# AIR-DISCOVER/Omni-PQ

Measured on AMD Instinct MI355X. Metric: scenes/sec fwd+bwd, 40k-pt ScanNet clouds, batch 8/GPU, higher is better.
Workload: dtype bf16; 1 GPU; BASELINE configs[1]: PQ_Transformer fwd+bwd, 40000-pt synthetic room scenes, batch 8/GPU, 3 input channels; global_batch=8, points=40000, parallelism=dp1, loss=sum of output means (SURVEY 8d)

## Files before the change

### include/omnipq_attn.h

```cpp
#ifndef OMNIPQ_ATTN_H
#define OMNIPQ_ATTN_H
#include "omnipq_pointops.h"

#ifdef __cplusplus
extern "C" {
#endif

int omnipq_attn_fwd(int N, int H, int L, int S, int D, const void *q, const void *k, const void *v, void *o,
                    const long long *strides, float *lse2, float dropout_p, const unsigned long long *seed_ptr,
                    unsigned salt, void *stream);

int omnipq_attn_bwd(int N, int H, int L, int S, int D, const void *q, const void *k, const void *v, const void *o,
                    const void *d_o, const long long *strides, const float *lse2, float *delta, void *dq, void *dk,
                    void *dv, const long long *grad_strides, float dropout_p, const unsigned long long *seed_ptr,
                    unsigned salt, void *stream);

int omnipq_attn_dropout_mask(int N, int H, int L, int S, float dropout_p, const unsigned long long *seed_ptr,
                             unsigned salt, unsigned char *mask, void *stream);

void omnipq_attn_block_map(int mode);

#ifdef __cplusplus
}
#endif
#endif
```

### omni-pq_amd/csrc/attention.hip

```cpp
#include "common.h"
#include "omnipq_attn.h"

namespace omnipq {

typedef float f32x16 __attribute__((ext_vector_type(16)));

constexpr int ATT_DMAX = 48;
constexpr int ATT_PITCH = 56;

struct AttnArgs {
  int N, H, L, S, D;
  long long q_sl, q_sn, k_sl, k_sn, v_sl, v_sn, o_sl, o_sn;
  float scale, scale_log2;
  float keep_inv;
  unsigned drop_thresh;
  unsigned salt;
  int xcd_map;
  const unsigned long long *seed_ptr;
};

__device__ __forceinline__ unsigned drop_seed(const AttnArgs &g) {
  if (!g.drop_thresh) return 0u;
  const unsigned long long s = *g.seed_ptr * 0x9E3779B97F4A7C15ull + 0xD1B54A32D192ED03ull * (g.salt + 1u);
  return (unsigned)(s >> 32) ^ (unsigned)s;
// ... 30 lines not shown
}

__device__ __forceinline__ float bf_lo(unsigned w) { return e16_lo(w); }
__device__ __forceinline__ float bf_hi(unsigned w) { return e16_hi(w); }

__device__ __forceinline__ float frag_dot(e16x8 a, e16x8 b) {
  const uint4 x = __builtin_bit_cast(uint4, a), y = __builtin_bit_cast(uint4, b);
  float s = bf_lo(x.x) * bf_lo(y.x) + bf_hi(x.x) * bf_hi(y.x);
  s += bf_lo(x.y) * bf_lo(y.y) + bf_hi(x.y) * bf_hi(y.y);
  s += bf_lo(x.z) * bf_lo(y.z) + bf_hi(x.z) * bf_hi(y.z);
  s += bf_lo(x.w) * bf_lo(y.w) + bf_hi(x.w) * bf_hi(y.w);
  return s;
}

__device__ __forceinline__ e16x8 pack_regs(const float *p, int j2) {
  e16x8 f;
#pragma unroll
  for (int e = 0; e < 8; ++e) f[e] = (e16_t)p[8 * j2 + e];
  return f;
}

constexpr int ATT_NP = 6;
constexpr int ATT_AREA = 33 * ATT_PITCH;
struct StagePlan {
  unsigned voff[ATT_NP];
  int lds[ATT_NP];
};

__device__ __forceinline__ StagePlan stage_plan(int D, int lane, long long s_tok) {
  StagePlan sp;
  const int ppr = D >> 2;
#pragma unroll
  for (int i = 0; i < ATT_NP; ++i) {
    const int id = lane + 64 * i;
    const int tok = id / ppr, off = (id - tok * ppr) * 4;
    const bool has = id < 32 * ppr;
    sp.voff[i] = has ? (unsigned)(tok * (int)s_tok + off) * 2u : ATT_OOB;
    sp.lds[i] = has ? tok * ATT_PITCH + off : 32 * ATT_PITCH;
  }
  return sp;
}

struct StageRegs {
  v2u v[ATT_NP];
};

__device__ __forceinline__ StageRegs stage_load(const StagePlan &sp, rsrc_t block) {
  StageRegs r;
#pragma unroll
  for (int i = 0; i < ATT_NP; ++i) r.v[i] = att_load8(block, sp.voff[i]);
  return r;
}

__device__ __forceinline__ void stage_store(const StagePlan &sp, const StageRegs &r, e16_t *lds) {
#pragma unroll
  for (int i = 0; i < ATT_NP; ++i) *reinterpret_cast<v2u *>(lds + sp.lds[i]) = r.v[i];
}

__device__ __forceinline__ void stage_clear(e16_t *lds, int areas, int lane) {
  for (int o = lane * 4; o < areas * ATT_AREA; o += 256) *reinterpret_cast<v2u *>(lds + o) = v2u{0u, 0u};
}

__device__ __forceinline__ e16x8 frag_lds_tok(const e16_t *lds, int row, int j, int h) {
  return *reinterpret_cast<const e16x8 *>(lds + row * ATT_PITCH + 16 * j + 8 * h);
}

typedef short v4s __attribute__((ext_vector_type(4)));
typedef __attribute__((address_space(3))) v4s lds_v4s;

__device__ __forceinline__ e16x8 frag_chan(const e16_t *lds, int t, int j2, int h, int lane) {
  const int grp = lane >> 4, l16 = lane & 15;
  int c0 = 32 * t + 16 * (grp & 1);
  c0 = c0 + 16 <= ATT_DMAX ? c0 : ATT_DMAX - 16;
  const e16_t *p = lds + (16 * j2 + 4 * h + (l16 >> 2)) * ATT_PITCH + c0 + (l16 & 3) * 4;
  const v4s lo = __builtin_amdgcn_ds_read_tr16_b64_v4i16((lds_v4s *)p);
  const v4s hi = __builtin_amdgcn_ds_read_tr16_b64_v4i16((lds_v4s *)(p + 8 * ATT_PITCH));
  return __builtin_bit_cast(e16x8, __builtin_shufflevector(lo, hi, 0, 1, 2, 3, 4, 5, 6, 7));
}

__device__ __forceinline__ float fast_exp2(float x) { return __builtin_amdgcn_exp2f(x); }

__device__ __forceinline__ float xor32(float v) { return __shfl_xor(v, 32, 64); }

__device__ __forceinline__ void att_block(const AttnArgs &g, int &blk, int &nh) {
  const int gx = (int)gridDim.x, gy = (int)gridDim.y;
  blk = (int)blockIdx.x, nh = (int)blockIdx.y;
  if (g.xcd_map && (gy & 7) == 0) {
    const int id = blk + gx * nh, slot = id >> 3;
    nh = (id & 7) + 8 * (slot / gx);
    blk = slot % gx;
  }
}

#define MFMA(a, b, c) mfma_e16_32x32x16(a, b, c)

__global__ __launch_bounds__(256) void attn_fwd_kernel(AttnArgs g, const e16_t *__restrict__ Q,
                                                      const e16_t *__restrict__ K, const e16_t *__restrict__ V,
                                                      e16_t *__restrict__ O, float *__restrict__ lse2) {
  __shared__ __attribute__((aligned(16))) unsigned char smem[4 * 64 * 33 * 4 + 4 * 32 * 4 * 2];
  const int tid = (int)threadIdx.x, lane = tid & 63, wave = __builtin_amdgcn_readfirstlane(tid >> 6), h = lane >> 5, ql = lane & 31;
  int blk, nh;
  att_block(g, blk, nh);
  const int n = nh / g.H, hd = nh - n * g.H;
  const int q0 = blk * 32, q = q0 + ql;
  const e16_t *Qb = Q + n * g.q_sn + hd * g.D, *Kb = K + n * g.k_sn + hd * g.D, *Vb = V + n * g.v_sn + hd * g.D;
  e16_t *ks = reinterpret_cast<e16_t *>(smem) + wave * 2 * ATT_AREA, *vs = ks + ATT_AREA;
  stage_clear(ks, 2, lane);

  e16x8 qf[3];
  {
    const rsrc_t rq = att_rsrc(Qb, g.q_sl, q0, g.L, g.D);
#pragma unroll
    for (int j = 0; j < 3; ++j) qf[j] = frag_tok(rq, (unsigned)(ql * (int)g.q_sl) * 2u, j, h, g.D);
  }

  const unsigned seed = drop_seed(g);
  float m = -1e30f, lsum = 0.f;
  f32x16 acc[2];
#pragma unroll
  for (int t = 0; t < 2; ++t)
#pragma unroll
    for (int r = 0; r < 16; ++r) acc[t][r] = 0.f;

  const int nkb = (g.S + 31) >> 5, iters = (nkb + 3) >> 2;
  const StagePlan spk = stage_plan(g.D, lane, g.k_sl), spv = stage_plan(g.D, lane, g.v_sl);
  StageRegs kn = stage_load(spk, att_rsrc(Kb, g.k_sl, wave * 32, g.S, g.D));
  StageRegs vn = stage_load(spv, att_rsrc(Vb, g.v_sl, wave * 32, g.S, g.D));
  for (int it = 0; it < iters; ++it) {
    const int k0 = (it * 4 + wave) * 32;
    const StageRegs kc = kn, vc = vn;
    if (it + 1 < iters) {
      kn = stage_load(spk, att_rsrc(Kb, g.k_sl, k0 + 128, g.S, g.D));
      vn = stage_load(spv, att_rsrc(Vb, g.v_sl, k0 + 128, g.S, g.D));
    }
    __builtin_amdgcn_fence(__ATOMIC_ACQ_REL, "wavefront");
    __builtin_amdgcn_wave_barrier();
    stage_store(spk, kc, ks);
    stage_store(spv, vc, vs);
    __builtin_amdgcn_fence(__ATOMIC_ACQ_REL, "wavefront");
    __builtin_amdgcn_wave_barrier();
    f32x16 st;
#pragma unroll
    for (int r = 0; r < 16; ++r) st[r] = 0.f;
#pragma unroll
    for (int j = 0; j < 3; ++j) st = MFMA(frag_lds_tok(ks, ql, j, h), qf[j], st);
    float p[16], bm = -1e30f;
    const bool full = k0 + 32 <= g.S;
    if (full) {
#pragma unroll
      for (int r = 0; r < 16; ++r) bm = fmaxf(bm, st[r]);
      bm *= g.scale_log2;
    } else {
#pragma unroll
      for (int r = 0; r < 16; ++r) {
        const bool ok = k0 + acc_row(r, h) < g.S;
        p[r] = ok ? st[r] * g.scale_log2 : -1e30f;
        bm = fmaxf(bm, p[r]);
      }
    }
    bm = fmaxf(bm, xor32(bm));
    const float m_new = fmaxf(m, bm);
    const float alpha = fast_exp2(m - m_new);
    float rs = 0.f;
    if (full) {
#pragma unroll
      for (int r = 0; r < 16; ++r) {
        p[r] = fast_exp2(__builtin_fmaf(st[r], g.scale_log2, -m_new));
        rs += p[r];
      }
    } else {
#pragma unroll
      for (int r = 0; r < 16; ++r) {
        const bool ok = k0 + acc_row(r, h) < g.S;
        p[r] = ok ? fast_exp2(p[r] - m_new) : 0.f;
        rs += p[r];
      }
    }
    rs += xor32(rs);
    lsum = lsum * alpha + rs;
    if (__builtin_amdgcn_ballot_w64(m_new != m) != 0) {
#pragma unroll
      for (int t = 0; t < 2; ++t)
#pragma unroll
        for (int r = 0; r < 16; ++r) acc[t][r] *= alpha;
    }
    m = m_new;
    if (g.drop_thresh) {
      const unsigned base = ((unsigned)nh * (unsigned)g.L + (unsigned)q) * (unsigned)g.S + (unsigned)k0 + seed + 4u * h;
#pragma unroll
      for (int r = 0; r < 16; ++r)
        p[r] = drop_hash_mix(base + (unsigned)acc_row(r, 0)) >= g.drop_thresh ? p[r] * g.keep_inv : 0.f;
    }
    __builtin_amdgcn_fence(__ATOMIC_ACQ_REL, "wavefront");
    __builtin_amdgcn_wave_barrier();
#pragma unroll
    for (int j2 = 0; j2 < 2; ++j2) {
      const e16x8 pf = pack_regs(p, j2);
#pragma unroll
      for (int t = 0; t < 2; ++t) acc[t] = MFMA(frag_chan(vs, t, j2, h, lane), pf, acc[t]);
    }
  }

  __syncthreads();
  float *ms = reinterpret_cast<float *>(smem + 4 * 64 * 33 * 4);
  float *comb = reinterpret_cast<float *>(smem);
  if (h == 0) ms[wave * 32 + ql] = m;
  __syncthreads();
  const float mstar = fmaxf(fmaxf(ms[ql], ms[32 + ql]), fmaxf(ms[64 + ql], ms[96 + ql]));
  const float f = fast_exp2(m - mstar);
  if (h == 0) ms[128 + wave * 32 + ql] = lsum * f;
#pragma unroll
  for (int t = 0; t < 2; ++t)
#pragma unroll
    for (int r = 0; r < 16; ++r) comb[(wave * 64 + 32 * t + acc_row(r, h)) * 33 + ql] = acc[t][r] * f;
  __syncthreads();
  for (int idx = tid; idx < 32 * g.D; idx += 256) {
    const int qq = idx / g.D, d = idx - qq * g.D;
    if (q0 + qq < g.L) {
      const float l = ms[128 + qq] + ms[160 + qq] + ms[192 + qq] + ms[224 + qq];
      const float o = comb[(0 * 64 + d) * 33 + qq] + comb[(1 * 64 + d) * 33 + qq] + comb[(2 * 64 + d) * 33 + qq] +
                      comb[(3 * 64 + d) * 33 + qq];
      O[(long long)(q0 + qq) * g.o_sl + n * g.o_sn + hd * g.D + d] = (e16_t)(o / l);
    }
  }
  if (tid < 32 && q0 + tid < g.L) {
    const float l = ms[128 + tid] + ms[160 + tid] + ms[192 + tid] + ms[224 + tid];
    const float ms_ = fmaxf(fmaxf(ms[tid], ms[32 + tid]), fmaxf(ms[64 + tid], ms[96 + tid]));
    lse2[(long long)nh * g.L + q0 + tid] = ms_ + log2f(l);
  }
}

__global__ __launch_bounds__(256) void attn_bwd_dq_kernel(AttnArgs g, const e16_t *__restrict__ Q,
                                                         const e16_t *__restrict__ K, const e16_t *__restrict__ V,
                                                         const e16_t *__restrict__ O, const e16_t *__restrict__ dO,
                                                         const float *__restrict__ lse2, float *__restrict__ delta,
                                                         e16_t *__restrict__ dQ, long long dq_sl, long long dq_sn) {
  __shared__ __attribute__((aligned(16))) unsigned char smem[4 * 64 * 33 * 4];
  const int tid = (int)threadIdx.x, lane = tid & 63, wave = __builtin_amdgcn_readfirstlane(tid >> 6), h = lane >> 5, ql = lane & 31;
  int blk, nh;
  att_block(g, blk, nh);
  const int n = nh / g.H, hd = nh - n * g.H;
  const int q0 = blk * 32, q = q0 + ql;
  const bool qv = q < g.L;
  const e16_t *Qb = Q + n * g.q_sn + hd * g.D, *Kb = K + n * g.k_sn + hd * g.D, *Vb = V + n * g.v_sn + hd * g.D;
  const e16_t *Ob = O + n * g.o_sn + hd * g.D, *dOb = dO + n * g.o_sn + hd * g.D;
  e16_t *ks = reinterpret_cast<e16_t *>(smem) + wave * 2 * ATT_AREA, *vs = ks + ATT_AREA;
  stage_clear(ks, 2, lane);

  e16x8 qf[3], dof[3];
  float dl = 0.f;
  {
    const rsrc_t rq = att_rsrc(Qb, g.q_sl, q0, g.L, g.D), ro = att_rsrc(Ob, g.o_sl, q0, g.L, g.D);
    const rsrc_t rdo = att_rsrc(dOb, g.o_sl, q0, g.L, g.D);
    const unsigned qoff = (unsigned)(ql * (int)g.q_sl) * 2u, ooff = (unsigned)(ql * (int)g.o_sl) * 2u;
#pragma unroll
    for (int j = 0; j < 3; ++j) {
      qf[j] = frag_tok(rq, qoff, j, h, g.D);
      dof[j] = frag_tok(rdo, ooff, j, h, g.D);
      dl += frag_dot(dof[j], frag_tok(ro, ooff, j, h, g.D));
    }
  }
  dl += xor32(dl);
  if (wave == 0 && h == 0 && qv) delta[(long long)nh * g.L + q] = dl;
  const float lse = qv ? lse2[(long long)nh * g.L + q] : 0.f;

  const unsigned seed = drop_seed(g);
  f32x16 acc[2];
#pragma unroll
  for (int t = 0; t < 2; ++t)
#pragma unroll
    for (int r = 0; r < 16; ++r) acc[t][r] = 0.f;

  const int nkb = (g.S + 31) >> 5, iters = (nkb + 3) >> 2;
  const StagePlan spk = stage_plan(g.D, lane, g.k_sl), spv = stage_plan(g.D, lane, g.v_sl);
  StageRegs kn = stage_load(spk, att_rsrc(Kb, g.k_sl, wave * 32, g.S, g.D));
  StageRegs vn = stage_load(spv, att_rsrc(Vb, g.v_sl, wave * 32, g.S, g.D));
  for (int it = 0; it < iters; ++it) {
    const int k0 = (it * 4 + wave) * 32;
    const StageRegs kc = kn, vc = vn;
    if (it + 1 < iters) {
      kn = stage_load(spk, att_rsrc(Kb, g.k_sl, k0 + 128, g.S, g.D));
      vn = stage_load(spv, att_rsrc(Vb, g.v_sl, k0 + 128, g.S, g.D));
    }
    __builtin_amdgcn_fence(__ATOMIC_ACQ_REL, "wavefront");
    __builtin_amdgcn_wave_barrier();
    stage_store(spk, kc, ks);
    stage_store(spv, vc, vs);
    __builtin_amdgcn_fence(__ATOMIC_ACQ_REL, "wavefront");
    __builtin_amdgcn_wave_barrier();
    f32x16 st, dp;
#pragma unroll
    for (int r = 0; r < 16; ++r) st[r] = dp[r] = 0.f;
#pragma unroll
    for (int j = 0; j < 3; ++j) {
      st = MFMA(frag_lds_tok(ks, ql, j, h), qf[j], st);
      dp = MFMA(frag_lds_tok(vs, ql, j, h), dof[j], dp);
    }
    float ds[16];
    const unsigned base = ((unsigned)nh * (unsigned)g.L + (unsigned)q) * (unsigned)g.S + (unsigned)k0 + seed + 4u * h;
    const bool full = q0 + 32 <= g.L && k0 + 32 <= g.S;
#pragma unroll
    for (int r = 0; r < 16; ++r) ds[r] = fast_exp2(__builtin_fmaf(st[r], g.scale_log2, -lse));
    if (!full) {
#pragma unroll
      for (int r = 0; r < 16; ++r) ds[r] = (qv && k0 + acc_row(r, h) < g.S) ? ds[r] : 0.f;
    }
    if (g.drop_thresh) {
#pragma unroll
      for (int r = 0; r < 16; ++r)
        dp[r] = drop_hash_mix(base + (unsigned)acc_row(r, 0)) >= g.drop_thresh ? dp[r] * g.keep_inv : 0.f;
    }
#pragma unroll
    for (int r = 0; r < 16; ++r) ds[r] *= dp[r] - dl;
#pragma unroll
    for (int j2 = 0; j2 < 2; ++j2) {
      const e16x8 df = pack_regs(ds, j2);
#pragma unroll
      for (int t = 0; t < 2; ++t) acc[t] = MFMA(frag_chan(ks, t, j2, h, lane), df, acc[t]);
    }
  }
  __syncthreads();
  float *comb = reinterpret_cast<float *>(smem);
#pragma unroll
  for (int t = 0; t < 2; ++t)
#pragma unroll
    for (int r = 0; r < 16; ++r) comb[(wave * 64 + 32 * t + acc_row(r, h)) * 33 + ql] = acc[t][r];
  __syncthreads();
  for (int idx = tid; idx < 32 * g.D; idx += 256) {
    const int qq = idx / g.D, d = idx - qq * g.D;
    if (q0 + qq < g.L) {
      const float v = comb[(0 * 64 + d) * 33 + qq] + comb[(1 * 64 + d) * 33 + qq] + comb[(2 * 64 + d) * 33 + qq] +
                      comb[(3 * 64 + d) * 33 + qq];
      dQ[(long long)(q0 + qq) * dq_sl + n * dq_sn + hd * g.D + d] = (e16_t)(v * g.scale);
    }
  }
}

__global__ __launch_bounds__(256) void attn_bwd_dkdv_kernel(AttnArgs g, const e16_t *__restrict__ Q,
                                                           const e16_t *__restrict__ K, const e16_t *__restrict__ V,
                                                           const e16_t *__restrict__ dO, const float *__restrict__ lse2,
                                                           const float *__restrict__ delta, e16_t *__restrict__ dK,
                                                           long long dk_sl, long long dk_sn, e16_t *__restrict__ dV,
                                                           long long dv_sl, long long dv_sn) {
  __shared__ __attribute__((aligned(16))) e16_t qs[2 * ATT_AREA];
  __shared__ float rowv[64];
  const int tid = (int)threadIdx.x, lane = tid & 63, wave = __builtin_amdgcn_readfirstlane(tid >> 6), h = lane >> 5, kl = lane & 31;
  int blk, nh;
  att_block(g, blk, nh);
  const int n = nh / g.H, hd = nh - n * g.H;
  const int kb0 = blk * 128, k0 = kb0 + wave * 32, key = k0 + kl;
  const bool kv = key < g.S;
  const e16_t *Qb = Q + n * g.q_sn + hd * g.D, *Kb = K + n * g.k_sn + hd * g.D, *Vb = V + n * g.v_sn + hd * g.D;
  const e16_t *dOb = dO + n * g.o_sn + hd * g.D;
  e16_t *dos = qs + ATT_AREA;
  for (int o = tid * 4; o < 2 * ATT_AREA; o += 1024) *reinterpret_cast<v2u *>(qs + o) = v2u{0u, 0u};

  e16x8 kf[3], vf[3];
  {
    const rsrc_t rk = att_rsrc(Kb, g.k_sl, kb0, g.S, g.D), rv = att_rsrc(Vb, g.v_sl, kb0, g.S, g.D);
    const unsigned koff = (unsigned)((wave * 32 + kl) * (int)g.k_sl) * 2u, voff = (unsigned)((wave * 32 + kl) * (int)g.v_sl) * 2u;
#pragma unroll
    for (int j = 0; j < 3; ++j) {
      kf[j] = frag_tok(rk, koff, j, h, g.D);
      vf[j] = frag_tok(rv, voff, j, h, g.D);
    }
  }
  const unsigned seed = drop_seed(g);
  f32x16 accv[2], acck[2];
#pragma unroll
  for (int t = 0; t < 2; ++t)
#pragma unroll
    for (int r = 0; r < 16; ++r) accv[t][r] = acck[t][r] = 0.f;

  const int ppr = g.D >> 2;
  unsigned qvo[2], dvo[2];
  int plds[2];
#pragma unroll
  for (int i = 0; i < 2; ++i) {
    const int id = tid + 256 * i, tok = id / ppr, off = (id - tok * ppr) * 4;
    const bool has = id < 32 * ppr;
    qvo[i] = has ? (unsigned)(tok * (int)g.q_sl + off) * 2u : ATT_OOB;
    dvo[i] = has ? (unsigned)(tok * (int)g.o_sl + off) * 2u : ATT_OOB;
    plds[i] = has ? tok * ATT_PITCH + off : 32 * ATT_PITCH;
  }
  const float *rowsrc = (tid < 32 ? lse2 : delta) + (long long)nh * g.L;
  v2u qn[2], dn[2];
  float rown = 0.f;
  auto fetch = [&](int q0) {
    const rsrc_t rq = att_rsrc(Qb, g.q_sl, q0, g.L, g.D), rdo = att_rsrc(dOb, g.o_sl, q0, g.L, g.D);
#pragma unroll
    for (int i = 0; i < 2; ++i) {
      qn[i] = att_load8(rq, qvo[i]);
      dn[i] = att_load8(rdo, dvo[i]);
    }
    rown = (tid < 64 && q0 + (tid & 31) < g.L) ? rowsrc[q0 + (tid & 31)] : 0.f;
  };
  fetch(0);
  const int nqb = (g.L + 31) >> 5;
  __syncthreads();
  for (int it = 0; it < nqb; ++it) {
    const int q0 = it * 32;
    v2u qc[2], dc[2];
#pragma unroll
    for (int i = 0; i < 2; ++i) qc[i] = qn[i], dc[i] = dn[i];
    const float rowc = rown;
    if (it + 1 < nqb) fetch(q0 + 32);
    __syncthreads();
#pragma unroll
    for (int i = 0; i < 2; ++i) {
      *reinterpret_cast<v2u *>(qs + plds[i]) = qc[i];
      *reinterpret_cast<v2u *>(dos + plds[i]) = dc[i];
    }
    if (tid < 64) rowv[tid] = rowc;
    __syncthreads();
    f32x16 s, dp;
#pragma unroll
    for (int r = 0; r < 16; ++r) s[r] = dp[r] = 0.f;
#pragma unroll
    for (int j = 0; j < 3; ++j) {
      s = MFMA(frag_lds_tok(qs, kl, j, h), kf[j], s);
      dp = MFMA(frag_lds_tok(dos, kl, j, h), vf[j], dp);
    }
    float pt[16], ds[16];
    const bool full = q0 + 32 <= g.L && k0 + 32 <= g.S;
    const unsigned hbase = ((unsigned)nh * (unsigned)g.L + (unsigned)(q0 + 4 * h)) * (unsigned)g.S + (unsigned)key + seed;
#pragma unroll
    for (int r = 0; r < 16; ++r) pt[r] = fast_exp2(__builtin_fmaf(s[r], g.scale_log2, -rowv[acc_row(r, h)]));
    if (!full) {
#pragma unroll
      for (int r = 0; r < 16; ++r) pt[r] = (kv && q0 + acc_row(r, h) < g.L) ? pt[r] : 0.f;
    }
#pragma unroll
    for (int r = 0; r < 16; ++r) ds[r] = pt[r];
    if (g.drop_thresh) {
#pragma unroll
      for (int r = 0; r < 16; ++r) {
        const float km = drop_hash_mix(hbase + (unsigned)acc_row(r, 0) * (unsigned)g.S) >= g.drop_thresh ? g.keep_inv : 0.f;
        dp[r] *= km;
        pt[r] *= km;
      }
    }
#pragma unroll
    for (int r = 0; r < 16; ++r) ds[r] *= dp[r] - rowv[32 + acc_row(r, h)];
#pragma unroll
    for (int j2 = 0; j2 < 2; ++j2) {
      const e16x8 pf = pack_regs(pt, j2), df = pack_regs(ds, j2);
#pragma unroll
      for (int t = 0; t < 2; ++t) {
        accv[t] = MFMA(pf, frag_chan(dos, t, j2, h, lane), accv[t]);
        acck[t] = MFMA(df, frag_chan(qs, t, j2, h, lane), acck[t]);
      }
    }
  }
#pragma unroll
  for (int t = 0; t < 2; ++t) {
    const int d = 32 * t + kl;
    if (d < g.D) {
#pragma unroll
      for (int r = 0; r < 16; ++r) {
        const int kk = k0 + acc_row(r, h);
        if (kk < g.S) {
          dV[(long long)kk * dv_sl + n * dv_sn + hd * g.D + d] = (e16_t)accv[t][r];
          dK[(long long)kk * dk_sl + n * dk_sn + hd * g.D + d] = (e16_t)(acck[t][r] * g.scale);
        }
      }
    }
  }
}

__global__ void attn_mask_kernel(AttnArgs g, unsigned char *__restrict__ mask) {
  const long long total = (long long)g.N * g.H * g.L * g.S;
  const unsigned seed = drop_seed(g);
  for (long long i = (long long)blockIdx.x * blockDim.x + threadIdx.x; i < total; i += (long long)gridDim.x * blockDim.x)
    mask[i] = !g.drop_thresh || drop_hash((unsigned)i, seed) >= g.drop_thresh;
}

static int g_attn_xcd_map = 1;

static int token_strides_ok(const long long *strides, int n, int L, int S, int D) {
  const long long tok = L > S ? L : S;
  for (int i = 0; i < 2 * n; i += 2) {
    const long long sl = strides[i];
    if (sl < 0) return OMNIPQ_EINVAL;
    if (((tok - 1) * sl + D) * 2 >= (1ll << 31) || 32 * sl * 2 >= (1ll << 31)) return OMNIPQ_ETOOLARGE;
  }
  return OMNIPQ_OK;
}

static int fill_args(AttnArgs &g, int N, int H, int L, int S, int D, const long long *strides, float dropout_p,
                     const unsigned long long *seed_ptr, unsigned salt) {
  if (N <= 0 || H <= 0 || L <= 0 || S <= 0 || D <= 0 || (D % 4) || D > ATT_DMAX) return OMNIPQ_EINVAL;
  if (!(dropout_p >= 0.f) || dropout_p >= 1.f || (dropout_p > 0.f && !seed_ptr)) return OMNIPQ_EINVAL;
  if ((long long)N * H * L * S >= (1ll << 32)) return OMNIPQ_ETOOLARGE;
  for (int i = 0; i < 8; ++i)
    if (strides[i] % 4) return OMNIPQ_EINVAL;
  {
    const int rc = token_strides_ok(strides, 4, L, S, D);
    if (rc) return rc;
  }
  g.N = N, g.H = H, g.L = L, g.S = S, g.D = D;
  g.q_sl = strides[0], g.q_sn = strides[1], g.k_sl = strides[2], g.k_sn = strides[3];
  g.v_sl = strides[4], g.v_sn = strides[5], g.o_sl = strides[6], g.o_sn = strides[7];
  g.scale = 1.0f / sqrtf((float)D);
  g.scale_log2 = g.scale * 1.4426950408889634f;
  g.keep_inv = 1.0f / (1.0f - dropout_p);
  double th = (double)dropout_p * 4294967296.0;
  g.drop_thresh = dropout_p > 0.f ? (unsigned)(th < 1.0 ? 1.0 : (th > 4294967295.0 ? 4294967295.0 : th)) : 0u;
  g.salt = salt;
  g.xcd_map = g_attn_xcd_map;
  g.seed_ptr = seed_ptr;
  return OMNIPQ_OK;
}

}

extern "C" void omnipq_attn_block_map(int mode) { omnipq::g_attn_xcd_map = mode ? 1 : 0; }

extern "C" int omnipq_attn_fwd(int N, int H, int L, int S, int D, const void *q, const void *k, const void *v,
                               void *o, const long long *strides, float *lse2, float dropout_p,
                               const unsigned long long *seed_ptr, unsigned salt, void *stream) {
  using namespace omnipq;
  AttnArgs g;
  if (!q || !k || !v || !o || !strides || !lse2) return OMNIPQ_EINVAL;
  const int rc = fill_args(g, N, H, L, S, D, strides, dropout_p, seed_ptr, salt);
  if (rc) return rc;
  attn_fwd_kernel<<<dim3((L + 31) / 32, N * H), 256, 0, (hipStream_t)stream>>>(
      g, (const e16_t *)q, (const e16_t *)k, (const e16_t *)v, (e16_t *)o, lse2);
  OMNIPQ_LAUNCH_CHECK();
  return OMNIPQ_OK;
}

extern "C" int omnipq_attn_bwd(int N, int H, int L, int S, int D, const void *q, const void *k, const void *v,
                               const void *o, const void *d_o, const long long *strides, const float *lse2,
                               float *delta, void *dq, void *dk, void *dv, const long long *grad_strides,
                               float dropout_p, const unsigned long long *seed_ptr, unsigned salt, void *stream) {
  using namespace omnipq;
  AttnArgs g;
  if (!q || !k || !v || !o || !d_o || !strides || !lse2 || !delta || !dq || !dk || !dv || !grad_strides)
    return OMNIPQ_EINVAL;
  const int rc = fill_args(g, N, H, L, S, D, strides, dropout_p, seed_ptr, salt);
  if (rc) return rc;
  for (int i = 0; i < 6; ++i)
    if (grad_strides[i] % 4) return OMNIPQ_EINVAL;
  if (const int rs = token_strides_ok(grad_strides, 3, L, S, D)) return rs;
  attn_bwd_dq_kernel<<<dim3((L + 31) / 32, N * H), 256, 0, (hipStream_t)stream>>>(
      g, (const e16_t *)q, (const e16_t *)k, (const e16_t *)v, (const e16_t *)o, (const e16_t *)d_o, lse2, delta,
      (e16_t *)dq, grad_strides[0], grad_strides[1]);
  OMNIPQ_LAUNCH_CHECK();
  attn_bwd_dkdv_kernel<<<dim3((S + 127) / 128, N * H), 256, 0, (hipStream_t)stream>>>(
      g, (const e16_t *)q, (const e16_t *)k, (const e16_t *)v, (const e16_t *)d_o, lse2, delta, (e16_t *)dk,
      grad_strides[2], grad_strides[3], (e16_t *)dv, grad_strides[4], grad_strides[5]);
  OMNIPQ_LAUNCH_CHECK();
  return OMNIPQ_OK;
}

extern "C" int omnipq_attn_dropout_mask(int N, int H, int L, int S, float dropout_p,
                                        const unsigned long long *seed_ptr, unsigned salt, unsigned char *mask,
                                        void *stream) {
  using namespace omnipq;
  AttnArgs g;
  const long long zero[8] = {0, 0, 0, 0, 0, 0, 0, 0};
  if (!mask) return OMNIPQ_EINVAL;
  const int rc = fill_args(g, N, H, L, S, 4, zero, dropout_p, seed_ptr, salt);
  if (rc) return rc;
  attn_mask_kernel<<<1024, 256, 0, (hipStream_t)stream>>>(g, mask);
  OMNIPQ_LAUNCH_CHECK();
  return OMNIPQ_OK;
}
```

### omni-pq_amd/models/decoder_rows.py

```python
import ctypes
import os

import torch

import dropout_state
import rows_mlp
import sa_fused
from sa_fused import E16, _call, _lib, _p, zeros_f32
from utils import fused_attention



class AddToBf16(torch.autograd.Function):

    @staticmethod
    def forward(ctx, a, b):
        ctx.e16 = E16.dtype
        out = torch.empty(a.shape, device=a.device, dtype=E16.dtype)
        _call(_lib.omnipq_add_to_e16, a, a.numel(), _p(a), int(a.dtype == torch.float32), _p(b),
              _p(out))
        ctx.a_dtype = a.dtype
        return out

    @staticmethod
# ... 205 lines not shown
    if pe_a.training != pe_b.training or not (rows_mlp.usable(x, sa, pe_a.training) and rows_mlp.usable(x, sb, pe_b.training)):
        return None
    return rows_mlp.run_pair(x, sa, x, sb, pe_a.training)


def key_side(layer, key, key_pos, mem16=None, k_pe=None):
    C = key.shape[1]
    ca = layer.multihead_attn
    if mem16 is None:
        mem16 = _rows(key).to(E16.dtype)
    if k_pe is None:
        k_pe = _rows(layer.cross_posembed(key_pos)).to(E16.dtype)
    mem_pe = AddToBf16.apply(mem16, k_pe)
    wq, wkv = torch.split(ca.in_proj_weight, [C, 2 * C])
    bq, bkv = torch.split(ca.in_proj_bias, [C, 2 * C])
    return rows_mlp.run(mem_pe, [rows_mlp.Layer(wkv, bkv)], layer.training), (wq, bq)


def precompute_key_sides(layers, key, key_pos):
    cur = torch.cuda.current_stream(key.device)
    side = _side_stream(key.device)
    side.wait_stream(cur)
    with torch.cuda.stream(side):
        mem = FanOut.apply(_rows(key).to(E16.dtype).contiguous(), len(layers))
        kvs = []
        k_pes = [None] * len(layers)
        if PAIR_KEY_EMBEDDINGS:
            for i in range(0, len(layers) - 1, 2):
                both = posembed_pair(layers[i].cross_posembed, layers[i + 1].cross_posembed, key_pos)
                if both is not None:
                    k_pes[i], k_pes[i + 1] = both
        for i, layer in enumerate(layers):
            kv = key_side(layer, key, key_pos, mem[i], k_pes[i])
            if _JOIN_PER_LAYER:
                done = torch.cuda.Event()
                done.record(side)
                kv = kv + (done,)
            kvs.append(kv)
    for kv in kvs:
        kv[0].record_stream(cur)
    return kvs


_JOIN_PER_LAYER = True
PAIR_KEY_EMBEDDINGS = True


def join_key_sides(device, done=None):
    if done is not None:
        torch.cuda.current_stream(device).wait_event(done)
    else:
        torch.cuda.current_stream(device).wait_stream(_side_stream(device))


def run(layer, query, key, query_pos, key_pos, kv=None):
    B, C, Pq = query.shape
    Pk = key.shape[2]
    training = layer.training
    sa, ca = layer.self_attn, layer.multihead_attn
    H = sa.num_heads
    p_attn = float(sa.dropout) if training else 0.0

    def pdrop(m):
        return float(m.p) if training else 0.0

    def linear(x, w, b, **kw):
        return rows_mlp.run(x, [rows_mlp.Layer(w, b, **kw)], training)

    x32 = _rows(query).float()
    q_pe = _rows(layer.self_posembed(query_pos)).to(E16.dtype)

    x16_in = getattr(query, "omnipq_rows16", None)
    if x16_in is not None and x16_in.is_contiguous() and tuple(x16_in.shape) == (B, Pq, C) and \
            x16_in.requires_grad == x32.requires_grad:
        qk = AddToBf16.apply(x16_in.view(B * Pq, C), q_pe)
    else:
        qk = AddToBf16.apply(x32, q_pe)
    qkv = linear(qk, sa.in_proj_weight, sa.in_proj_bias)
    att = fused_attention.PackedAttention.apply(qkv, None, Pq, Pq, B, H, p_attn)
    y = linear(att, sa.out_proj.weight, sa.out_proj.bias)
    x32, _, xq = AddDropoutLayerNorm.apply(x32, y, layer.norm1.weight, layer.norm1.bias, float(layer.norm1.eps),
                                           pdrop(layer.dropout1), q_pe, True, False)

    if kv is None:
        kv = key_side(layer, key, key_pos)
    else:
        join_key_sides(query.device, kv[2] if len(kv) > 2 else None)
    kv, (wq, bq) = kv[0], kv[1]
    q = linear(xq, wq, bq)
    att = fused_attention.PackedAttention.apply(q, kv, Pq, Pk, B, H, float(ca.dropout) if training else 0.0)
    y = linear(att, ca.out_proj.weight, ca.out_proj.bias)
    x32, x16, _ = AddDropoutLayerNorm.apply(x32, y, layer.norm2.weight, layer.norm2.bias, float(layer.norm2.eps),
                                            pdrop(layer.dropout2), None, True, True)

    y = rows_mlp.run(x16, [rows_mlp.Layer(layer.linear1.weight, layer.linear1.bias, relu_dropout=pdrop(layer.dropout)),
                           rows_mlp.Layer(layer.linear2.weight, layer.linear2.bias)], training)
    x32, x16, _ = AddDropoutLayerNorm.apply(x32, y, layer.norm3.weight, layer.norm3.bias, float(layer.norm3.eps),
                                            pdrop(layer.dropout3), None, True, True)
    out = x32.view(B, Pq, C).transpose(1, 2)
    out.omnipq_rows16 = x16.view(B, Pq, C)
    return out
```

### omni-pq_amd/models/utils/fused_attention.py

```python
import ctypes

import torch

import sa_fused
from sa_fused import E16, _call, _lib, _p

MAX_HEAD_DIM = 48


from dropout_state import STATE


def usable(q, k, v, num_heads):
    E = q.shape[-1]
    if not (q.is_cuda and q.dtype == k.dtype == v.dtype == E16.dtype):
        return False
    D = E // num_heads
    if D * num_heads != E or D % 4 or D > MAX_HEAD_DIM:
        return False
    for t in (q, k, v):
        if t.dim() != 3 or t.stride(2) != 1 or t.stride(0) % 4 or t.stride(1) % 4:
            return False
    return q.shape[1] * num_heads * q.shape[0] * k.shape[0] < 2 ** 32


def _strides(*tensors):
    vals = []
    for t in tensors:
        vals += [t.stride(0), t.stride(1)]
    return (ctypes.c_longlong * len(vals))(*vals)


class FusedAttention(torch.autograd.Function):

    @staticmethod
    def forward(ctx, q, k, v, num_heads, dropout_p):
        ctx.e16 = E16.dtype
        L, N, E = q.shape
        S = k.shape[0]
        D = E // num_heads
        o = torch.empty((L, N, E), device=q.device, dtype=E16.dtype)
        lse = torch.empty((N * num_heads, L), device=q.device, dtype=torch.float32)
        seed = STATE.seed(q.device) if dropout_p > 0 else None
        salt = STATE.next_salt() if dropout_p > 0 else 0
        _call(_lib.omnipq_attn_fwd, q, N, num_heads, L, S, D, _p(q), _p(k), _p(v), _p(o), _strides(q, k, v, o), _p(lse),
              dropout_p, _p(seed), salt)
        ctx.save_for_backward(q, k, v, o, lse)
        ctx.cfg = (num_heads, dropout_p, seed, salt)
        return o

    @staticmethod
    def backward(ctx, d_o):
        E16.select(ctx.e16)
        q, k, v, o, lse = ctx.saved_tensors
        num_heads, dropout_p, seed, salt = ctx.cfg
        L, N, E = q.shape
        S = k.shape[0]
        D = E // num_heads
        d_o = d_o.to(E16.dtype)
        if d_o.stride() != o.stride():
            d_o = d_o.contiguous()
        dq = torch.empty((L, N, E), device=q.device, dtype=E16.dtype)
        dk = torch.empty((S, N, E), device=q.device, dtype=E16.dtype)
        dv = torch.empty((S, N, E), device=q.device, dtype=E16.dtype)
        delta = torch.empty_like(lse)
        _call(_lib.omnipq_attn_bwd, q, N, num_heads, L, S, D, _p(q), _p(k), _p(v), _p(o), _p(d_o),
              _strides(q, k, v, o), _p(lse), _p(delta), _p(dq), _p(dk), _p(dv), _strides(dq, dk, dv),
              dropout_p, _p(seed), salt)
        return dq, dk, dv, None, None


def attention(q, k, v, num_heads, dropout_p):
    return FusedAttention.apply(q, k, v, num_heads, float(dropout_p))


def dropout_mask(N, H, L, S, dropout_p, seed, salt):
    mask = torch.empty((N * H, L, S), device=seed.device, dtype=torch.uint8)
    _call(_lib.omnipq_attn_dropout_mask, mask, N, H, L, S, dropout_p, _p(seed), salt, _p(mask))
    return mask


class PackedAttention(torch.autograd.Function):

    @staticmethod
    def _pointers(a, b, E, L, S):
        if b is None:
            base = a.data_ptr()
            return (base, base + 2 * E, base + 4 * E), [3 * E, L * 3 * E] * 3
        kb = b.data_ptr()
        return (a.data_ptr(), kb, kb + 2 * E), [E, L * E, 2 * E, S * 2 * E, 2 * E, S * 2 * E]

    @staticmethod
    def forward(ctx, a, b, L, S, N, H, dropout_p):
        ctx.e16 = E16.dtype
        E = a.shape[1] // 3 if b is None else a.shape[1]
        D = E // H
        (qp, kp, vp), st = PackedAttention._pointers(a, b, E, L, S)
        o = torch.empty((N * L, E), device=a.device, dtype=E16.dtype)
        lse = torch.empty((N * H, L), device=a.device, dtype=torch.float32)
        seed = STATE.seed(a.device) if dropout_p > 0 else None
        salt = STATE.next_salt() if dropout_p > 0 else 0
        strides = (ctypes.c_longlong * 8)(*(st + [E, L * E]))
        _call(_lib.omnipq_attn_fwd, a, N, H, L, S, D, ctypes.c_void_p(qp), ctypes.c_void_p(kp), ctypes.c_void_p(vp),
              _p(o), strides, _p(lse), dropout_p, _p(seed), salt)
        ctx.save_for_backward(a, b, o, lse)
        ctx.cfg = (L, S, N, H, dropout_p, seed, salt)
        return o

    @staticmethod
    def backward(ctx, d_o):
        E16.select(ctx.e16)
        a, b, o, lse = ctx.saved_tensors
        L, S, N, H, dropout_p, seed, salt = ctx.cfg
        E = o.shape[1]
        D = E // H
        d_o = d_o.to(E16.dtype).contiguous()
        (qp, kp, vp), st = PackedAttention._pointers(a, b, E, L, S)
        da = torch.empty_like(a)
        db = torch.empty_like(b) if b is not None else None
        (dqp, dkp, dvp), gst = PackedAttention._pointers(da, db, E, L, S)
        delta = torch.empty_like(lse)
        strides = (ctypes.c_longlong * 8)(*(st + [E, L * E]))
        gstrides = (ctypes.c_longlong * 6)(*gst)
        _call(_lib.omnipq_attn_bwd, a, N, H, L, S, D, ctypes.c_void_p(qp), ctypes.c_void_p(kp), ctypes.c_void_p(vp),
              _p(o), _p(d_o), strides, _p(lse), _p(delta), ctypes.c_void_p(dqp), ctypes.c_void_p(dkp),
              ctypes.c_void_p(dvp), gstrides, dropout_p, _p(seed), salt)
        return da, db, None, None, None, None, None


def packed_usable(a, b, H):
    E = a.shape[1] // 3 if b is None else a.shape[1]
    D = E // H
    ok = a.is_cuda and a.dtype == E16.dtype and a.is_contiguous() and D * H == E and D % 4 == 0 and D <= MAX_HEAD_DIM
    if b is not None:
        ok = ok and b.dtype == E16.dtype and b.is_contiguous() and b.shape[1] == 2 * E
    return ok
```

Measured before the change: 1032 scenes/s.

## Merge attention backward dQ and dK/dV into one launch with inline delta

Attention backward now runs as a single grid whose first blocks compute dK/dV and whose remaining blocks compute dQ. The dK/dV path recomputes the row delta (dO·O) itself instead of waiting for the dQ kernel to write it. This removes one launch and the serial dependency between the two kernels so they can fill the GPU together, at the cost of redundant delta work and extra O loads and LDS in the dK/dV blocks. It also adds an option, off by default, to run cross-attention dK/dV on a side stream.

```diff
diff --git a/include/omnipq_attn.h b/include/omnipq_attn.h
--- a/include/omnipq_attn.h
+++ b/include/omnipq_attn.h
@@ -15,6 +15,18 @@
                     void *dv, const long long *grad_strides, float dropout_p, const unsigned long long *seed_ptr,
                     unsigned salt, void *stream);
 
+int omnipq_attn_bwd_dq(int N, int H, int L, int S, int D, const void *q, const void *k, const void *v, const void *o,
+                       const void *d_o, const long long *strides, const float *lse2, float *delta, void *dq,
+                       const long long *grad_strides, float dropout_p, const unsigned long long *seed_ptr, unsigned salt,
+                       void *stream);
+
+int omnipq_attn_bwd_dkdv(int N, int H, int L, int S, int D, const void *q, const void *k, const void *v, const void *o,
+                         const void *d_o, const long long *strides, const float *lse2, void *dk, void *dv,
+                         const long long *grad_strides, float dropout_p, const unsigned long long *seed_ptr, unsigned salt,
+                         void *stream);
+
+void omnipq_attn_bwd_mode(int mode);
+
 int omnipq_attn_dropout_mask(int N, int H, int L, int S, float dropout_p, const unsigned long long *seed_ptr,
                              unsigned salt, unsigned char *mask, void *stream);
 
diff --git a/omni-pq_amd/csrc/attention.hip b/omni-pq_amd/csrc/attention.hip
--- a/omni-pq_amd/csrc/attention.hip
+++ b/omni-pq_amd/csrc/attention.hip
@@ -136,14 +136,21 @@
 
 __device__ __forceinline__ float xor32(float v) { return __shfl_xor(v, 32, 64); }
 
+__device__ __forceinline__ void att_block_of(const AttnArgs &g, int id, int gx, int gy, int &blk, int &nh) {
+  if (g.xcd_map && (gy & 7) == 0) {
+    const int slot = id >> 3;
+    nh = (id & 7) + 8 * (slot / gx);
+    blk = slot % gx;
+  } else {
+    nh = id / gx;
+    blk = id - nh * gx;
+  }
+}
+
 __device__ __forceinline__ void att_block(const AttnArgs &g, int &blk, int &nh) {
   const int gx = (int)gridDim.x, gy = (int)gridDim.y;
   blk = (int)blockIdx.x, nh = (int)blockIdx.y;
-  if (g.xcd_map && (gy & 7) == 0) {
-    const int id = blk + gx * nh, slot = id >> 3;
-    nh = (id & 7) + 8 * (slot / gx);
-    blk = slot % gx;
-  }
+  if (g.xcd_map && (gy & 7) == 0) att_block_of(g, blk + gx * nh, gx, gy, blk, nh);
 }
 
 #define MFMA(a, b, c) mfma_e16_32x32x16(a, b, c)
@@ -284,15 +291,13 @@
   }
 }
 
-__global__ __launch_bounds__(256) void attn_bwd_dq_kernel(AttnArgs g, const e16_t *__restrict__ Q,
-                                                         const e16_t *__restrict__ K, const e16_t *__restrict__ V,
-                                                         const e16_t *__restrict__ O, const e16_t *__restrict__ dO,
-                                                         const float *__restrict__ lse2, float *__restrict__ delta,
-                                                         e16_t *__restrict__ dQ, long long dq_sl, long long dq_sn) {
-  __shared__ __attribute__((aligned(16))) unsigned char smem[4 * 64 * 33 * 4];
+__device__ __forceinline__ void attn_bwd_dq_program(const AttnArgs &g, int blk, int nh, unsigned char *smem,
+                                                    const e16_t *__restrict__ Q, const e16_t *__restrict__ K,
+                                                    const e16_t *__restrict__ V, const e16_t *__restrict__ O,
+                                                    const e16_t *__restrict__ dO, const float *__restrict__ lse2,
+                                                    float *__restrict__ delta, e16_t *__restrict__ dQ, long long dq_sl,
+                                                    long long dq_sn) {
   const int tid = (int)threadIdx.x, lane = tid & 63, wave = __builtin_amdgcn_readfirstlane(tid >> 6), h = lane >> 5, ql = lane & 31;
-  int blk, nh;
-  att_block(g, blk, nh);
   const int n = nh / g.H, hd = nh - n * g.H;
   const int q0 = blk * 32, q = q0 + ql;
   const bool qv = q < g.L;
@@ -390,24 +395,46 @@
   }
 }
 
-__global__ __launch_bounds__(256) void attn_bwd_dkdv_kernel(AttnArgs g, const e16_t *__restrict__ Q,
-                                                           const e16_t *__restrict__ K, const e16_t *__restrict__ V,
-                                                           const e16_t *__restrict__ dO, const float *__restrict__ lse2,
-                                                           const float *__restrict__ delta, e16_t *__restrict__ dK,
-                                                           long long dk_sl, long long dk_sn, e16_t *__restrict__ dV,
-                                                           long long dv_sl, long long dv_sn) {
-  __shared__ __attribute__((aligned(16))) e16_t qs[2 * ATT_AREA];
-  __shared__ float rowv[64];
-  const int tid = (int)threadIdx.x, lane = tid & 63, wave = __builtin_amdgcn_readfirstlane(tid >> 6), h = lane >> 5, kl = lane & 31;
+constexpr int ATT_DQ_SMEM = 4 * 64 * 33 * 4;
+
+__global__ __launch_bounds__(256) void attn_bwd_dq_kernel(AttnArgs g, const e16_t *__restrict__ Q,
+                                                         const e16_t *__restrict__ K, const e16_t *__restrict__ V,
+                                                         const e16_t *__restrict__ O, const e16_t *__restrict__ dO,
+                                                         const float *__restrict__ lse2, float *__restrict__ delta,
+                                                         e16_t *__restrict__ dQ, long long dq_sl, long long dq_sn) {
+  __shared__ __attribute__((aligned(16))) unsigned char smem[ATT_DQ_SMEM];
   int blk, nh;
   att_block(g, blk, nh);
+  attn_bwd_dq_program(g, blk, nh, smem, Q, K, V, O, dO, lse2, delta, dQ, dq_sl, dq_sn);
+}
+
+template <bool DELTA_IN>
+struct DkdvSmem {
+  static constexpr int areas = DELTA_IN ? 2 : 3;
+  static constexpr int rows = DELTA_IN ? 64 : 32 + 4 * 32;
+  static constexpr int bytes = areas * ATT_AREA * 2 + rows * 4;
+};
+
+template <bool DELTA_IN>
+__device__ __forceinline__ void attn_bwd_dkdv_program(const AttnArgs &g, int blk, int nh, unsigned char *smem,
+                                                      const e16_t *__restrict__ Q, const e16_t *__restrict__ K,
+                                                      const e16_t *__restrict__ V, const e16_t *__restrict__ O,
+                                                      const e16_t *__restrict__ dO, const float *__restrict__ lse2,
+                                                      const float *__restrict__ delta, e16_t *__restrict__ dK,
+                                                      long long dk_sl, long long dk_sn, e16_t *__restrict__ dV,
+                                                      long long dv_sl, long long dv_sn) {
+  constexpr int AREAS = DkdvSmem<DELTA_IN>::areas;
+  e16_t *qs = reinterpret_cast<e16_t *>(smem);
+  float *rowv = reinterpret_cast<float *>(smem + AREAS * ATT_AREA * 2);
+  const int tid = (int)threadIdx.x, lane = tid & 63, wave = __builtin_amdgcn_readfirstlane(tid >> 6), h = lane >> 5, kl = lane & 31;
   const int n = nh / g.H, hd = nh - n * g.H;
   const int kb0 = blk * 128, k0 = kb0 + wave * 32, key = k0 + kl;
   const bool kv = key < g.S;
   const e16_t *Qb = Q + n * g.q_sn + hd * g.D, *Kb = K + n * g.k_sn + hd * g.D, *Vb = V + n * g.v_sn + hd * g.D;
-  const e16_t *dOb = dO + n * g.o_sn + hd * g.D;
-  e16_t *dos = qs + ATT_AREA;
-  for (int o = tid * 4; o < 2 * ATT_AREA; o += 1024) *reinterpret_cast<v2u *>(qs + o) = v2u{0u, 0u};
+  const e16_t *dOb = dO + n * g.o_sn + hd * g.D, *Ob = DELTA_IN ? dOb : O + n * g.o_sn + hd * g.D;
+  e16_t *dos = qs + ATT_AREA, *os = qs + (AREAS - 1) * ATT_AREA;
+  float *rowd = DELTA_IN ? rowv + 32 : rowv + 32 + wave * 32;
+  for (int o = tid * 4; o < AREAS * ATT_AREA; o += 1024) *reinterpret_cast<v2u *>(qs + o) = v2u{0u, 0u};
 
   e16x8 kf[3], vf[3];
   {
@@ -437,8 +464,9 @@
     dvo[i] = has ? (unsigned)(tok * (int)g.o_sl + off) * 2u : ATT_OOB;
     plds[i] = has ? tok * ATT_PITCH + off : 32 * ATT_PITCH;
   }
-  const float *rowsrc = (tid < 32 ? lse2 : delta) + (long long)nh * g.L;
-  v2u qn[2], dn[2];
+  constexpr int NROW = DELTA_IN ? 64 : 32;
+  const float *rowsrc = (tid < 32 || !DELTA_IN ? lse2 : delta) + (long long)nh * g.L;
+  v2u qn[2], dn[2], on[2];
   float rown = 0.f;
   auto fetch = [&](int q0) {
     const rsrc_t rq = att_rsrc(Qb, g.q_sl, q0, g.L, g.D), rdo = att_rsrc(dOb, g.o_sl, q0, g.L, g.D);
@@ -447,16 +475,24 @@
       qn[i] = att_load8(rq, qvo[i]);
       dn[i] = att_load8(rdo, dvo[i]);
     }
-    rown = (tid < 64 && q0 + (tid & 31) < g.L) ? rowsrc[q0 + (tid & 31)] : 0.f;
+    if (!DELTA_IN) {
+      const rsrc_t ro = att_rsrc(Ob, g.o_sl, q0, g.L, g.D);
+#pragma unroll
+      for (int i = 0; i < 2; ++i) on[i] = att_load8(ro, dvo[i]);
+    }
+    rown = (tid < NROW && q0 + (tid & 31) < g.L) ? rowsrc[q0 + (tid & 31)] : 0.f;
   };
   fetch(0);
   const int nqb = (g.L + 31) >> 5;
   __syncthreads();
   for (int it = 0; it < nqb; ++it) {
     const int q0 = it * 32;
-    v2u qc[2], dc[2];
-#pragma unroll
-    for (int i = 0; i < 2; ++i) qc[i] = qn[i], dc[i] = dn[i];
+    v2u qc[2], dc[2], oc[2];
+#pragma unroll
+    for (int i = 0; i < 2; ++i) {
+      qc[i] = qn[i], dc[i] = dn[i];
+      if (!DELTA_IN) oc[i] = on[i];
+    }
     const float rowc = rown;
     if (it + 1 < nqb) fetch(q0 + 32);
     __syncthreads();
@@ -464,8 +500,9 @@
     for (int i = 0; i < 2; ++i) {
       *reinterpret_cast<v2u *>(qs + plds[i]) = qc[i];
       *reinterpret_cast<v2u *>(dos + plds[i]) = dc[i];
-    }
-    if (tid < 64) rowv[tid] = rowc;
+      if (!DELTA_IN) *reinterpret_cast<v2u *>(os + plds[i]) = oc[i];
+    }
+    if (tid < NROW) rowv[tid] = rowc;
     __syncthreads();
     f32x16 s, dp;
 #pragma unroll
@@ -474,6 +511,17 @@
     for (int j = 0; j < 3; ++j) {
       s = MFMA(frag_lds_tok(qs, kl, j, h), kf[j], s);
       dp = MFMA(frag_lds_tok(dos, kl, j, h), vf[j], dp);
+    }
+    if (!DELTA_IN) {
+      float dl = 0.f;
+#pragma unroll
+      for (int j = 0; j < 3; ++j) dl += frag_dot(frag_lds_tok(dos, kl, j, h), frag_lds_tok(os, kl, j, h));
+      dl += xor32(dl);
+      __builtin_amdgcn_fence(__ATOMIC_ACQ_REL, "wavefront");
+      __builtin_amdgcn_wave_barrier();
+      if (h == 0) rowd[kl] = dl;
+      __builtin_amdgcn_fence(__ATOMIC_ACQ_REL, "wavefront");
+      __builtin_amdgcn_wave_barrier();
     }
     float pt[16], ds[16];
     const bool full = q0 + 32 <= g.L && k0 + 32 <= g.S;
@@ -495,7 +543,7 @@
       }
     }
 #pragma unroll
-    for (int r = 0; r < 16; ++r) ds[r] *= dp[r] - rowv[32 + acc_row(r, h)];
+    for (int r = 0; r < 16; ++r) ds[r] *= dp[r] - rowd[acc_row(r, h)];
 #pragma unroll
     for (int j2 = 0; j2 < 2; ++j2) {
       const e16x8 pf = pack_regs(pt, j2), df = pack_regs(ds, j2);
@@ -519,6 +567,40 @@
         }
       }
     }
+  }
+}
+
+template <bool DELTA_IN>
+__global__ __launch_bounds__(256) void attn_bwd_dkdv_kernel(AttnArgs g, const e16_t *__restrict__ Q,
+                                                           const e16_t *__restrict__ K, const e16_t *__restrict__ V,
+                                                           const e16_t *__restrict__ O, const e16_t *__restrict__ dO,
+                                                           const float *__restrict__ lse2, const float *__restrict__ delta,
+                                                           e16_t *__restrict__ dK, long long dk_sl, long long dk_sn,
+                                                           e16_t *__restrict__ dV, long long dv_sl, long long dv_sn) {
+  __shared__ __attribute__((aligned(16))) unsigned char smem[DkdvSmem<DELTA_IN>::bytes];
+  int blk, nh;
+  att_block(g, blk, nh);
+  attn_bwd_dkdv_program<DELTA_IN>(g, blk, nh, smem, Q, K, V, O, dO, lse2, delta, dK, dk_sl, dk_sn, dV, dv_sl, dv_sn);
+}
+
+__global__ __launch_bounds__(256) void attn_bwd_kernel(AttnArgs g, const e16_t *__restrict__ Q, const e16_t *__restrict__ K,
+                                                      const e16_t *__restrict__ V, const e16_t *__restrict__ O,
+                                                      const e16_t *__restrict__ dO, const float *__restrict__ lse2,
+                                                      float *__restrict__ delta, e16_t *__restrict__ dQ, long long dq_sl,
+                                                      long long dq_sn, e16_t *__restrict__ dK, long long dk_sl,
+                                                      long long dk_sn, e16_t *__restrict__ dV, long long dv_sl,
+                                                      long long dv_sn) {
+  static_assert(DkdvSmem<false>::bytes <= ATT_DQ_SMEM, "one buffer of the larger size");
+  __shared__ __attribute__((aligned(16))) unsigned char smem[ATT_DQ_SMEM];
+  const int gy = (int)gridDim.y, gk = (g.S + 127) >> 7, gq = (int)gridDim.x - gk;
+  const int id = (int)blockIdx.x + (int)gridDim.x * (int)blockIdx.y;
+  int blk, nh;
+  if (id < gk * gy) {
+    att_block_of(g, id, gk, gy, blk, nh);
+    attn_bwd_dkdv_program<false>(g, blk, nh, smem, Q, K, V, O, dO, lse2, nullptr, dK, dk_sl, dk_sn, dV, dv_sl, dv_sn);
+  } else {
+    att_block_of(g, id - gk * gy, gq, gy, blk, nh);
+    attn_bwd_dq_program(g, blk, nh, smem, Q, K, V, O, dO, lse2, delta, dQ, dq_sl, dq_sn);
   }
 }
 
@@ -584,6 +666,20 @@
   return OMNIPQ_OK;
 }
 
+namespace omnipq {
+
+static int g_attn_bwd_mode = 1;
+
+static int grad_strides_ok(const long long *gs, int n, int L, int S, int D) {
+  for (int i = 0; i < 2 * n; ++i)
+    if (gs[i] % 4) return OMNIPQ_EINVAL;
+  return token_strides_ok(gs, n, L, S, D);
+}
+
+}
+
+extern "C" void omnipq_attn_bwd_mode(int mode) { omnipq::g_attn_bwd_mode = mode ? 1 : 0; }
+
 extern "C" int omnipq_attn_bwd(int N, int H, int L, int S, int D, const void *q, const void *k, const void *v,
                                const void *o, const void *d_o, const long long *strides, const float *lse2,
                                float *delta, void *dq, void *dk, void *dv, const long long *grad_strides,
@@ -594,16 +690,57 @@
     return OMNIPQ_EINVAL;
   const int rc = fill_args(g, N, H, L, S, D, strides, dropout_p, seed_ptr, salt);
   if (rc) return rc;
-  for (int i = 0; i < 6; ++i)
-    if (grad_strides[i] % 4) return OMNIPQ_EINVAL;
-  if (const int rs = token_strides_ok(grad_strides, 3, L, S, D)) return rs;
+  if (const int rs = grad_strides_ok(grad_strides, 3, L, S, D)) return rs;
+  const int gq = (L + 31) / 32, gk = (S + 127) / 128;
+  if (g_attn_bwd_mode) {
+    attn_bwd_kernel<<<dim3(gk + gq, N * H), 256, 0, (hipStream_t)stream>>>(
+        g, (const e16_t *)q, (const e16_t *)k, (const e16_t *)v, (const e16_t *)o, (const e16_t *)d_o, lse2, delta,
+        (e16_t *)dq, grad_strides[0], grad_strides[1], (e16_t *)dk, grad_strides[2], grad_strides[3], (e16_t *)dv,
+        grad_strides[4], grad_strides[5]);
+    OMNIPQ_LAUNCH_CHECK();
+    return OMNIPQ_OK;
+  }
+  attn_bwd_dq_kernel<<<dim3(gq, N * H), 256, 0, (hipStream_t)stream>>>(
+      g, (const e16_t *)q, (const e16_t *)k, (const e16_t *)v, (const e16_t *)o, (const e16_t *)d_o, lse2, delta,
+      (e16_t *)dq, grad_strides[0], grad_strides[1]);
+  OMNIPQ_LAUNCH_CHECK();
+  attn_bwd_dkdv_kernel<true><<<dim3(gk, N * H), 256, 0, (hipStream_t)stream>>>(
+      g, (const e16_t *)q, (const e16_t *)k, (const e16_t *)v, nullptr, (const e16_t *)d_o, lse2, delta, (e16_t *)dk,
+      grad_strides[2], grad_strides[3], (e16_t *)dv, grad_strides[4], grad_strides[5]);
+  OMNIPQ_LAUNCH_CHECK();
+  return OMNIPQ_OK;
+}
+
+extern "C" int omnipq_attn_bwd_dq(int N, int H, int L, int S, int D, const void *q, const void *k, const void *v,
+                                  const void *o, const void *d_o, const long long *strides, const float *lse2,
+                                  float *delta, void *dq, const long long *grad_strides, float dropout_p,
+                                  const unsigned long long *seed_ptr, unsigned salt, void *stream) {
+  using namespace omnipq;
+  AttnArgs g;
+  if (!q || !k || !v || !o || !d_o || !strides || !lse2 || !delta || !dq || !grad_strides) return OMNIPQ_EINVAL;
+  const int rc = fill_args(g, N, H, L, S, D, strides, dropout_p, seed_ptr, salt);
+  if (rc) return rc;
+  if (const int rs = grad_strides_ok(grad_strides, 1, L, S, D)) return rs;
   attn_bwd_dq_kernel<<<dim3((L + 31) / 32, N * H), 256, 0, (hipStream_t)stream>>>(
       g, (const e16_t *)q, (const e16_t *)k, (const e16_t *)v, (const e16_t *)o, (const e16_t *)d_o, lse2, delta,
       (e16_t *)dq, grad_strides[0], grad_strides[1]);
   OMNIPQ_LAUNCH_CHECK();
-  attn_bwd_dkdv_kernel<<<dim3((S + 127) / 128, N * H), 256, 0, (hipStream_t)stream>>>(
-      g, (const e16_t *)q, (const e16_t *)k, (const e16_t *)v, (const e16_t *)d_o, lse2, delta, (e16_t *)dk,
-      grad_strides[2], grad_strides[3], (e16_t *)dv, grad_strides[4], grad_strides[5]);
+  return OMNIPQ_OK;
+}
+
+extern "C" int omnipq_attn_bwd_dkdv(int N, int H, int L, int S, int D, const void *q, const void *k, const void *v,
+                                    const void *o, const void *d_o, const long long *strides, const float *lse2, void *dk,
+                                    void *dv, const long long *grad_strides, float dropout_p,
+                                    const unsigned long long *seed_ptr, unsigned salt, void *stream) {
+  using namespace omnipq;
+  AttnArgs g;
+  if (!q || !k || !v || !o || !d_o || !strides || !lse2 || !dk || !dv || !grad_strides) return OMNIPQ_EINVAL;
+  const int rc = fill_args(g, N, H, L, S, D, strides, dropout_p, seed_ptr, salt);
+  if (rc) return rc;
+  if (const int rs = grad_strides_ok(grad_strides, 2, L, S, D)) return rs;
+  attn_bwd_dkdv_kernel<false><<<dim3((S + 127) / 128, N * H), 256, 0, (hipStream_t)stream>>>(
+      g, (const e16_t *)q, (const e16_t *)k, (const e16_t *)v, (const e16_t *)o, (const e16_t *)d_o, lse2, nullptr,
+      (e16_t *)dk, grad_strides[0], grad_strides[1], (e16_t *)dv, grad_strides[2], grad_strides[3]);
   OMNIPQ_LAUNCH_CHECK();
   return OMNIPQ_OK;
 }
diff --git a/omni-pq_amd/models/decoder_rows.py b/omni-pq_amd/models/decoder_rows.py
--- a/omni-pq_amd/models/decoder_rows.py
+++ b/omni-pq_amd/models/decoder_rows.py
@@ -311,13 +311,15 @@
     x32, _, xq = AddDropoutLayerNorm.apply(x32, y, layer.norm1.weight, layer.norm1.bias, float(layer.norm1.eps),
                                            pdrop(layer.dropout1), q_pe, True, False)
 
+    kv_stream = None
     if kv is None:
         kv = key_side(layer, key, key_pos)
     else:
         join_key_sides(query.device, kv[2] if len(kv) > 2 else None)
+        kv_stream = _side_stream(query.device)
     kv, (wq, bq) = kv[0], kv[1]
     q = linear(xq, wq, bq)
-    att = fused_attention.PackedAttention.apply(q, kv, Pq, Pk, B, H, float(ca.dropout) if training else 0.0)
+    att = fused_attention.PackedAttention.apply(q, kv, Pq, Pk, B, H, float(ca.dropout) if training else 0.0, kv_stream)
     y = linear(att, ca.out_proj.weight, ca.out_proj.bias)
     x32, x16, _ = AddDropoutLayerNorm.apply(x32, y, layer.norm2.weight, layer.norm2.bias, float(layer.norm2.eps),
                                             pdrop(layer.dropout2), None, True, True)
diff --git a/omni-pq_amd/models/utils/fused_attention.py b/omni-pq_amd/models/utils/fused_attention.py
--- a/omni-pq_amd/models/utils/fused_attention.py
+++ b/omni-pq_amd/models/utils/fused_attention.py
@@ -6,6 +6,7 @@
 from sa_fused import E16, _call, _lib, _p
 
 MAX_HEAD_DIM = 48
+CROSS_DKDV_SIDE = False
 
 
 from dropout_state import STATE
@@ -91,8 +92,9 @@
         return (a.data_ptr(), kb, kb + 2 * E), [E, L * E, 2 * E, S * 2 * E, 2 * E, S * 2 * E]
 
     @staticmethod
-    def forward(ctx, a, b, L, S, N, H, dropout_p):
+    def forward(ctx, a, b, L, S, N, H, dropout_p, kv_stream=None):
         ctx.e16 = E16.dtype
+        ctx.kv_stream = kv_stream if b is not None else None
         E = a.shape[1] // 3 if b is None else a.shape[1]
         D = E // H
         (qp, kp, vp), st = PackedAttention._pointers(a, b, E, L, S)
@@ -117,15 +119,27 @@
         d_o = d_o.to(E16.dtype).contiguous()
         (qp, kp, vp), st = PackedAttention._pointers(a, b, E, L, S)
         da = torch.empty_like(a)
-        db = torch.empty_like(b) if b is not None else None
-        (dqp, dkp, dvp), gst = PackedAttention._pointers(da, db, E, L, S)
         delta = torch.empty_like(lse)
         strides = (ctypes.c_longlong * 8)(*(st + [E, L * E]))
-        gstrides = (ctypes.c_longlong * 6)(*gst)
-        _call(_lib.omnipq_attn_bwd, a, N, H, L, S, D, ctypes.c_void_p(qp), ctypes.c_void_p(kp), ctypes.c_void_p(vp),
-              _p(o), _p(d_o), strides, _p(lse), _p(delta), ctypes.c_void_p(dqp), ctypes.c_void_p(dkp),
-              ctypes.c_void_p(dvp), gstrides, dropout_p, _p(seed), salt)
-        return da, db, None, None, None, None, None
+        ptrs = (ctypes.c_void_p(qp), ctypes.c_void_p(kp), ctypes.c_void_p(vp), _p(o), _p(d_o), strides, _p(lse))
+        side = ctx.kv_stream if CROSS_DKDV_SIDE else None
+        if side is None:
+            db = torch.empty_like(b) if b is not None else None
+            (dqp, dkp, dvp), gst = PackedAttention._pointers(da, db, E, L, S)
+            _call(_lib.omnipq_attn_bwd, a, N, H, L, S, D, *ptrs, _p(delta), ctypes.c_void_p(dqp), ctypes.c_void_p(dkp),
+                  ctypes.c_void_p(dvp), (ctypes.c_longlong * 6)(*gst), dropout_p, _p(seed), salt)
+            return da, db, None, None, None, None, None, None
+        side.wait_stream(torch.cuda.current_stream(a.device))
+        with torch.cuda.stream(side):
+            db = torch.empty_like(b)
+            (_, dkp, dvp), gst = PackedAttention._pointers(da, db, E, L, S)
+            _call(_lib.omnipq_attn_bwd_dkdv, a, N, H, L, S, D, *ptrs, ctypes.c_void_p(dkp), ctypes.c_void_p(dvp),
+                  (ctypes.c_longlong * 4)(*gst[2:]), dropout_p, _p(seed), salt)
+        for t in (a, b, o, d_o, lse):
+            t.record_stream(side)
+        _call(_lib.omnipq_attn_bwd_dq, a, N, H, L, S, D, *ptrs, _p(delta), _p(da), (ctypes.c_longlong * 2)(*gst[:2]),
+              dropout_p, _p(seed), salt)
+        return da, db, None, None, None, None, None, None
 
 
 def packed_usable(a, b, H):
```

Result: faster. 1047 scenes/s (median of 6 runs) (+1.4%).
